# danielSanchezQ/dkg

Hardware: AMD Instinct MI355X
Metric: verified shares/sec (whole node) at n=1024,t=511; full-ceremony wall time (higher is better)
Workload: dtype u32 (GF(2^255-19), Z_l); 1 GPU; one DKG ceremony n=1024, t=511 (share gen + round-2/4 checks + finalise); n=1024, t=511, parallelism=single GPU, verify_streams=2, rounds_2_4_fused=True, degree_split=4, recombination=short lattice multipliers, recombination_addends=affine Niels, stepping_additions=dedicated (complete redo where exceptional)

## Files before the change

dkg_amd/_lib.py:

```python
import ctypes
import os
import sys

HERE = os.path.dirname(os.path.abspath(__file__))
LIB_PATH = os.environ.get("DKG_AMD_LIB", os.path.join(HERE, "libdkg_amd.so"))

DKG_OK = 0
DKG_E_ARG = -1
DKG_E_DECODE = -2
DKG_E_DEVICE = -3
DKG_E_NOMEM = -4
REJECT, ACCEPT, SELF, SKIPPED, MISSING = 0, 1, 2, 3, 4
FIN_OK, FIN_R2_ERROR, FIN_R4_ERROR, FIN_PHASE4_ERROR, FIN_INSUFFICIENT, FIN_PANIC = 0, 1, 2, 3, 4, 5
COMPLAINT_IGNORED, COMPLAINT_NO_PHASE3 = 4, 5

_lib = None


class DkgError(RuntimeError):
    def __init__(self, code, msg=""):
        self.code = code
        names = {DKG_E_ARG: "DKG_E_ARG", DKG_E_DECODE: "DKG_E_DECODE", DKG_E_DEVICE: "DKG_E_DEVICE",
                 DKG_E_NOMEM: "DKG_E_NOMEM"}
        super().__init__(f"{names.get(code, code)}: {msg}")
# ... 130 lines not shown
    L.dkg_ceremony_verify_fetched_proven.argtypes = [p, sz, sz, u8p, u8p, u8p, u8p, u8p, u8p, sz, p, p, u8p, u8p,
                                                     ctypes.POINTER(CeremonyOut), p, p, p]
    L.dkg_ceremony_verify_full_proven.argtypes = [p, sz, sz, u8p, u8p, u8p, u8p, u8p, u8p, sz, p, p, u8p, u8p, sz, p, p,
                                                  u8p, u8p, ctypes.POINTER(CeremonyOut), p, p, p, p, p]
    L.dkg_ceremony_batch_verify_proven.argtypes = [p, sz, sz, sz, u8p, u8p, u8p, u8p, u8p, u8p, sz, p, p, p, u8p, u8p,
                                                   ctypes.POINTER(BatchOut), p, p, p]
    L.dkg_ceremony_batch_verify_full_proven.argtypes = [p, sz, sz, sz, u8p, u8p, u8p, u8p, u8p, u8p, sz, p, p, p, u8p,
                                                        u8p, sz, p, p, p, u8p, u8p, ctypes.POINTER(BatchOut), p, p, p, p,
                                                        p, p, p]
    L.dkg_dealer_coeffs.argtypes = [u8p, ctypes.c_uint32, sz, sz, sz, p, p]
    L.dkg_scalar_sum_device.argtypes = [p, sz, sz, p, p, p]
    L.dkg_point_sum_device.argtypes = [p, sz, p, p, p]
    L.dkg_share_gen_device.argtypes = [p, sz, sz, sz, p, p, p, p, p, p]
    L.dkg_ceremony_shard_recon_device.argtypes = [p, sz, sz, sz, sz, u8p, u8p, u8p, u8p, p, p,
                                                  ctypes.POINTER(ctypes.c_int32)]
    L.dkg_finalise_parties.argtypes = [p, sz, sz, u8p, u8p, u8p, u8p, u8p, u8p, u8p, p, p, p]
    L.dkg_shard_range.argtypes = [sz, sz, sz, ctypes.POINTER(sz), ctypes.POINTER(sz)]
    L.dkg_shard_range.restype = None
    L.dkg_shard_rows.argtypes = [sz, sz]
    L.dkg_shard_rows.restype = sz
    L.dkg_shard_combine_device.argtypes = [p, sz, sz, sz, p, p, p, p, ctypes.POINTER(ShardOutcome)]
    L.dkg_shard_combine_packed_device.argtypes = [p, sz, sz, sz, p, p, p, p, ctypes.POINTER(ShardOutcome)]
    L.dkg_fixed_base_windows.argtypes = []
    L.dkg_key_comb_windows.argtypes = []
    L.dkg_packed_row_words.argtypes = [sz]
    L.dkg_packed_row_words.restype = sz
    L.dkg_decisions_pack_device.argtypes = [p, sz, sz, sz, sz, p, p]
    L.dkg_shard_finalise_device.argtypes = [p, sz, sz, sz, p, p, u8p, ctypes.c_int, p, p, p]
    L.dkg_multi_create.argtypes = [ctypes.POINTER(ctypes.c_int), ctypes.c_int, ctypes.POINTER(p)]
    L.dkg_multi_destroy.argtypes = [p]
    L.dkg_multi_destroy.restype = None
    L.dkg_multi_size.argtypes = [p]
    L.dkg_multi_ctx.argtypes = [p, ctypes.c_int]
    L.dkg_multi_ctx.restype = p
    L.dkg_multi_last_error.argtypes = [p]
    L.dkg_multi_last_error.restype = ctypes.c_char_p
    L.dkg_multi_phase_ms.argtypes = [p, ctypes.c_char_p]
    L.dkg_multi_phase_ms.restype = ctypes.c_double
    L.dkg_multi_env_init.argtypes = [p, sz, sz, u8p, sz, p]
    L.dkg_multi_ceremony_run.argtypes = [p, sz, sz, u8p, u8p, ctypes.POINTER(CeremonyOut)]
    L.dkg_multi_ceremony_run_device.argtypes = [p, sz, sz, ctypes.POINTER(p), ctypes.POINTER(p),
                                                ctypes.POINTER(CeremonyOut)]
    L.dkg_multi_ceremony_verify.argtypes = [p, sz, sz, u8p, u8p, u8p, u8p, ctypes.POINTER(CeremonyOut)]
    _lib = L
    return L


EXPORTED = [
    "dkg_ctx_create", "dkg_ctx_destroy", "dkg_ctx_last_error", "dkg_ctx_phase_ms", "dkg_ctx_set_streams", "dkg_ctx_set_overlap",
    "dkg_device_count", "dkg_env_init",
    "dkg_env_check", "dkg_msm_batch", "dkg_fixed_base_batch", "dkg_poly_eval_batch",
    "dkg_points_valid_batch", "dkg_share_gen", "dkg_verify_pairs", "dkg_verify_receiver",
    "dkg_ctx_set_split", "dkg_ctx_set_stepping", "dkg_ctx_set_field_mode", "dkg_ctx_set_binomial", "dkg_ctx_set_check", "dkg_ctx_last_split", "dkg_ctx_last_split_len", "dkg_ctx_set_verify_mode", "dkg_ctx_fallback_rows", "dkg_split_model_ms", "dkg_split_len",
    "dkg_ctx_set_combine", "dkg_ctx_last_combine", "dkg_ctx_last_binomial", "dkg_ctx_set_addends", "dkg_ctx_set_stepping_formula", "dkg_ctx_stepping_redos", "dkg_ctx_binomial_reruns", "dkg_split_multipliers", "dkg_jsf_digits", "dkg_split_digits",
    "dkg_ctx_clock_probe", "dkg_device_pci_bus_id",
    "dkg_ceremony_run", "dkg_ceremony_verify", "dkg_ceremony_verify_fetched", "dkg_ceremony_run_device", "dkg_ceremony_shard_device",
    "dkg_ceremony_shard_verify_device",
    "dkg_ceremony_batch_device", "dkg_ceremony_batch_verify", "dkg_member_keys", "dkg_enc_randomness",
    "dkg_enc_randomness_device", "dkg_encrypt_shares", "dkg_decrypt_shares", "dkg_ceremony_run_full_device",
    "dkg_ceremony_verify_full", "dkg_misbehaviour_prove", "dkg_complaint1_verify", "dkg_complaint3_verify", "dkg_dealer_coeffs", "dkg_dealer_coeffs_device",
    "dkg_scalar_sum_device", "dkg_point_sum_device", "dkg_ceremony_shard_recon_device", "dkg_finalise_parties",
    "dkg_share_gen_device", "dkg_shard_range", "dkg_shard_rows", "dkg_shard_combine_device",
    "dkg_shard_combine_packed_device", "dkg_packed_row_words", "dkg_fixed_base_windows", "dkg_key_comb_windows", "dkg_decisions_pack_device",
    "dkg_shard_finalise_device", "dkg_multi_create", "dkg_multi_destroy", "dkg_multi_size", "dkg_multi_ctx",
    "dkg_multi_last_error", "dkg_multi_phase_ms", "dkg_multi_env_init", "dkg_multi_ceremony_run",
    "dkg_multi_ceremony_run_device", "dkg_multi_ceremony_verify",
    "dkg_member_keys_batch", "dkg_encrypt_shares_batch", "dkg_decrypt_shares_batch", "dkg_ceremony_batch_full_device",
    "dkg_ceremony_batch_verify_full", "dkg_ctx_set_batch_full_chunk",
    "dkg_complaints_prove", "dkg_complaints_verify", "dkg_ctx_set_complaint_eval", "dkg_ceremony_verify_full_complaints",
    "dkg_complaints3_verify", "dkg_ceremony_verify_fetched_proven", "dkg_ceremony_verify_full_proven",
    "dkg_ceremony_batch_verify_proven", "dkg_ceremony_batch_verify_full_proven",
]
```

dkg_amd/csrc/kernels.h:

```cpp
#pragma once
#include <hip/hip_runtime.h>
#include <stddef.h>
#include <stdint.h>

#include "kernels_decl.inc"
```

dkg_amd/csrc/kernels.hip:

```cpp
#ifdef DKG_FE_ILP
#define dkgk dkgk_ilp
#endif
#include "kernels.h"
#include "split.h"

#include <algorithm>
#include <cmath>
#include "points.h"

namespace dkgk {

constexpr int COMB_WORDS = AFF_WORDS * COMB_ENTRIES;

#ifndef DKG_DECODE_WAVES
#define DKG_DECODE_WAVES 2
#endif
__global__ __launch_bounds__(256, DKG_DECODE_WAVES) void k_decode(const uint32_t* __restrict__ comp, size_t count,
                                                uint32_t* __restrict__ ext, size_t stride,
                                                uint8_t* __restrict__ ok, size_t pm_N, size_t pm_npad,
                                                uint32_t nseg, uint32_t seg, size_t pm_L, size_t pm_pstride) {
  size_t e = (size_t)blockIdx.x * blockDim.x + threadIdx.x;
  if (e >= count) return;
  uint32_t w[8];
  ld_words8(w, comp + 8 * e);
// ... 760 lines not shown
}

void binomial_wave_redo(size_t width, size_t npad, size_t N, const uint32_t* C, uint32_t* e, hipStream_t stream,
                        size_t pieces, size_t pstride, size_t last_len, uint32_t* flags, size_t col_base,
                        size_t dreal, unsigned gw) {
  const int last_off = (last_len && last_len < N) ? (int)(N - last_len) : 0;
  hipLaunchKernelGGL((k_binom_wave<true, false, false>), dim3((unsigned)(width / 64 * pieces)), dim3(64), 0, stream,
                     (int)N, npad, C, e, pstride, (unsigned)(width / 64), (unsigned)(pieces - 1), last_off, nullptr,
                     flags, col_base, dreal, gw ? gw : 64u);
}

uint32_t* binomial(size_t width, size_t npad, size_t N, const uint32_t* C, uint32_t* e0, uint32_t* e1,
                   hipStream_t stream, size_t pieces, size_t pstride, size_t last_len) {
  binom_init(width, npad, N, C, e0, stream, pieces, pstride);
  uint32_t* in = e0;
  uint32_t* out = e1;
  for (size_t r = 1; r < N; r++) {
    binom_step(r, width, npad, N, C, in, out, stream, pieces, pstride, last_len);
    std::swap(in, out);
  }
  return in;
}


__global__ __launch_bounds__(256) void k_to_column_major(size_t width, size_t npad, size_t N,
                                                         const uint32_t* __restrict__ e, uint32_t* __restrict__ eT,
                                                         size_t pstride) {
  __shared__ uint32_t tile[64][65];
  const size_t w = blockIdx.z % PT_WORDS, base = (blockIdx.z / PT_WORDS) * pstride;
  const size_t c0 = (size_t)blockIdx.x * 64, p0 = (size_t)blockIdx.y * 64;
  const size_t S = N * npad;
  const int tx = threadIdx.x & 63, ty = threadIdx.x >> 6;
#pragma unroll
  for (int i = 0; i < 16; i++) {
    const size_t p = p0 + ty + 4 * i, c = c0 + tx;
    if (p < N && c < width) tile[ty + 4 * i][tx] = e[w * S + p * npad + base + c];
  }
  __syncthreads();
#pragma unroll
  for (int i = 0; i < 16; i++) {
    const size_t c = c0 + ty + 4 * i, p = p0 + tx;
    if (p < N && c < width) eT[w * S + (base + c) * N + p] = tile[tx][ty + 4 * i];
  }
}

void to_column_major(size_t width, size_t npad, size_t N, const uint32_t* e, uint32_t* eT, size_t pieces,
                     size_t pstride, hipStream_t stream) {
  if (!width || !N) return;
  hipLaunchKernelGGL(k_to_column_major,
                     dim3((unsigned)((width + 63) / 64), (unsigned)((N + 63) / 64), (unsigned)(pieces * PT_WORDS)),
                     dim3(256), 0, stream, width, npad, N, e, eT, pstride);
}

template <int MAXBS, bool DED, bool PARTS>
__global__ __launch_bounds__(MAXBS) __attribute__((amdgpu_waves_per_eu(4, 4))) void k_stepping(
    size_t ndealers, size_t npad, size_t N, const uint32_t* __restrict__ e, size_t nrecv, size_t pos0, int P,
    const uint32_t* __restrict__ up,
    uint32_t* __restrict__ down,
    uint32_t* __restrict__ R, size_t pstride, size_t Nlive, unsigned piece0, int nseg, int Plast,
    uint32_t* __restrict__ flags, size_t col0, size_t dreal, unsigned gw, uint32_t* __restrict__ Rz, size_t j0,
    size_t j1, const uint32_t* __restrict__ sin, uint32_t* __restrict__ sout, size_t nin, size_t nout) {
  const size_t wg = (size_t)blockIdx.y * gridDim.x + blockIdx.x;
  if (!DED && flags && !flags[wg]) return;
  __shared__ uint32_t cols[PT_WORDS * MAXBS];
  const int l = threadIdx.x, bs = blockDim.x;
  const int Ncol = (nseg - 1) * P + Plast;
  const int slot = l / Ncol, p = l - slot * Ncol;
  const int sg = min(p / P, nseg - 1), q = p - sg * P;
  const int Pseg = sg == nseg - 1 ? Plast : P;
  const size_t dl = (size_t)blockIdx.x * (bs / Ncol) + slot;
  const bool live = slot < bs / Ncol && dl < ndealers;
  const size_t gcol = col0 + dl;
  const bool real = live && (gcol / gw) * 64 + (gcol % gw) % 64 < dreal;
  const size_t d = (blockIdx.y + piece0 + sg) * pstride + dl;
  const size_t S = N * npad;
  const size_t pos = pos0 + q;
  ge_p3 D;
  if (live && pos < Nlive) {
    if (PARTS && j0) pt_load(D, sin, nin * npad, d * nin + pos);
    else pt_load(D, e, S, d * N + pos);
  } else {
    ge_identity(D);
  }
  const bool top_lane = live && (q == Pseg - 1);
  const uint4* upd = (up && live) ? reinterpret_cast<const uint4*>(up + d * nrecv * PT_WORDS) : nullptr;
  uint4* downd = (down && live) ? reinterpret_cast<uint4*>(down + d * nrecv * PT_WORDS) : nullptr;
  uint32_t* mine = cols + l;
  uint32_t* base = cols + (l - q);
  const uint32_t* nbr = base + ((q + 1) % Pseg);
  bool bad = false;
  const size_t jbeg = PARTS ? j0 : 0, jend = PARTS ? j1 : nrecv;
  for (size_t j = jbeg; j < jend; j++) {
    {
      ge_cached c0;
      if (DED) ge_to_cached_ded(c0, D);
      else ge_to_cached(c0, D);
      if (q == 0) {
        if (downd) {
          const uint4* w4 = reinterpret_cast<const uint4*>(&c0);
#pragma unroll
          for (int k = 0; k < PT_WORDS / 4; k++) downd[j * (PT_WORDS / 4) + k] = w4[k];
        }
      } else {
        lds_put_cached(mine, c0, MAXBS);
      }
    }
    if (top_lane && upd) {
      ge_cached u;
      uint4* u4 = reinterpret_cast<uint4*>(&u);
#pragma unroll
      for (int k = 0; k < PT_WORDS / 4; k++) u4[k] = upd[j * (PT_WORDS / 4) + k];
      lds_put_cached(base, u, MAXBS);
    }
    __syncthreads();
    if (live && pos + 1 < Nlive && (q + 1 < Pseg || up) && pos + j < nrecv) {
      if (DED) {
        ge_add_ded_lds(D, D, nbr, MAXBS);
        bad |= real && fe_tight_zero(D.Z);
      } else {
        ge_add_lds(D, D, nbr, false, MAXBS);
      }
    }
    __syncthreads();
    if (live && q == 0 && R) {
      pt_store_aos<DKG_STEP_NT != 0>(R, d * nrecv + j, D);
      if (Rz) {
        uint2* z2 = reinterpret_cast<uint2*>(Rz + (d * nrecv + j) * 10);
#pragma unroll
        for (int k = 0; k < 5; k++) {
          if (DKG_STEP_NT) __builtin_nontemporal_store(D.Z.v[2 * k], reinterpret_cast<uint32_t*>(z2 + k));
          if (DKG_STEP_NT) __builtin_nontemporal_store(D.Z.v[2 * k + 1], reinterpret_cast<uint32_t*>(z2 + k) + 1);
          if (!DKG_STEP_NT) z2[k] = make_uint2(D.Z.v[2 * k], D.Z.v[2 * k + 1]);
        }
      }
    }
  }
  if constexpr (PARTS) {
    if (j1 < nrecv) {
      size_t dd = d;
      int qq = q;
      asm volatile("" : "+v"(dd), "+v"(qq));
      if (live && pos0 + qq < Nlive && pos0 + qq < nout) pt_store(sout, nout * npad, dd * nout + pos0 + qq, D);
    }
  }
  if (DED && bad) flags[wg] = 1u;
}

double step_occupancy(size_t bs, size_t maxbs) {
  const double wgs = std::min(std::floor(160.0 * 1024 / (160.0 * maxbs)), std::floor(16.0 / (bs / 64.0)));
  const double wps = wgs * (bs / 64.0) / 4.0;
  return wps >= 4 ? 1.0 : (wps >= 3 ? 0.85 + 0.15 * (wps - 3) : 0.7);
}

StepShape stepping_shape(size_t N) {
  StepShape sh;
  if (N > 512) {
    sh.nblk = (N + 511) / 512;
    sh.P = (N + sh.nblk - 1) / sh.nblk;
    sh.per = 1;
    sh.bs = (sh.P + 63) / 64 * 64;
    sh.maxbs = 512;
    return sh;
  }
  double best = -1;
  for (size_t maxbs : {256, 192, 512}) {
    if (maxbs < N) continue;
    StepShape o;
    o.nblk = 1;
    o.P = N;
    o.per = maxbs / N;
    o.bs = (o.per * N + 63) / 64 * 64;
    o.maxbs = maxbs;
    const double score = (double)(o.per * N) / o.bs * step_occupancy(o.bs, maxbs);
    if (score > best + 0.02) {
      best = score;
      sh = o;
    }
  }
  return sh;
}

bool stepping_whole_columns(size_t L, size_t pieces, size_t last_len) {
  return pieces > 1 && (pieces - 1) * L + last_len <= 512;
}

double stepping_cycles(size_t cols, size_t N, size_t pieces, size_t last_len, bool whole) {
  const double THR = 4.5, LAT = 8, SIMDS = 1024;
  if (!last_len || last_len > N) last_len = N;
  auto launch = [&](const StepShape& s, double np) {
    const double per_cu = std::min(std::floor(1024.0 / s.maxbs), std::floor(16.0 / (s.bs / 64.0)));
    const double wgs = std::ceil((double)cols / s.per) * np * s.nblk, cap = 256 * per_cu;
    const double rounds = std::ceil(wgs / cap), in_round = wgs / rounds;
    const double w = in_round * (s.bs / 64.0) / SIMDS;
    const double occ = std::min(1.0, std::max(0.7, 0.7 + 0.15 * (w - 2)));
    return rounds * std::max(w * THR / occ, LAT);
  };
  if (whole && stepping_whole_columns(N, pieces, last_len)) return launch(stepping_shape((pieces - 1) * N + last_len), 1);
  const StepShape sh = stepping_shape(N);
  if (sh.nblk > 1 || last_len == N) return launch(sh, (double)pieces);
  return (pieces > 1 ? launch(sh, (double)(pieces - 1)) : 0.0) + launch(stepping_shape(last_len), 1);
}

double stepping_waves_per_simd(size_t cols, size_t N, size_t pieces, size_t last_len, bool whole) {
  if (!last_len || last_len > N) last_len = N;
  const bool wc = whole && stepping_whole_columns(N, pieces, last_len);
  const StepShape s = stepping_shape(wc ? (pieces - 1) * N + last_len : N);
  const double np = wc ? 1.0 : (last_len == N || s.nblk > 1 ? (double)pieces : (double)(pieces - 1));
  const double per_cu = std::min(std::floor(1024.0 / s.maxbs), std::floor(16.0 / (s.bs / 64.0)));
  const double wgs = std::ceil((double)cols / s.per) * np * s.nblk, cap = 256 * per_cu;
  return wgs / std::ceil(wgs / cap) * (s.bs / 64.0) / 1024;
}

constexpr size_t TAIL_MAX_PHASES = 8;
size_t stepping_flag_words(size_t ndealers, size_t pieces) {
  return ndealers * (pieces == 1 ? TAIL_MAX_PHASES : pieces + 1);
}

struct ColReal {
  size_t col0, dreal;
  unsigned gw;
  uint32_t* Rz;
};

template <bool DED, bool PARTS>
void step_launch_p(int maxbs, dim3 grid, dim3 block, hipStream_t stream, size_t ndealers, size_t npad, size_t N,
                   const uint32_t* e, size_t nrecv, size_t pos0, int P, const uint32_t* up, uint32_t* down,
                   uint32_t* R, size_t pstride, size_t Nlive, unsigned piece0, int nseg, int Plast, uint32_t* flags,
                   const ColReal& cr, size_t j0, size_t j1, const uint32_t* sin, uint32_t* sout, size_t nin,
                   size_t nout) {
  if (maxbs == 192)
    hipLaunchKernelGGL((k_stepping<192, DED, PARTS>), grid, block, 0, stream, ndealers, npad, N, e, nrecv, pos0, P,
                       up, down, R, pstride, Nlive, piece0, nseg, Plast, flags, cr.col0, cr.dreal, cr.gw,
                       R ? cr.Rz : nullptr, j0, j1, sin, sout, nin, nout);
  else if (maxbs == 256)
    hipLaunchKernelGGL((k_stepping<256, DED, PARTS>), grid, block, 0, stream, ndealers, npad, N, e, nrecv, pos0, P,
                       up, down, R, pstride, Nlive, piece0, nseg, Plast, flags, cr.col0, cr.dreal, cr.gw,
                       R ? cr.Rz : nullptr, j0, j1, sin, sout, nin, nout);
  else
    hipLaunchKernelGGL((k_stepping<512, DED, PARTS>), grid, block, 0, stream, ndealers, npad, N, e, nrecv, pos0, P,
                       up, down, R, pstride, Nlive, piece0, nseg, Plast, flags, cr.col0, cr.dreal, cr.gw,
                       R ? cr.Rz : nullptr, j0, j1, sin, sout, nin, nout);
}

template <bool DED>
void step_launch(int maxbs, dim3 grid, dim3 block, hipStream_t stream, size_t ndealers, size_t npad, size_t N,
                 const uint32_t* e, size_t nrecv, size_t pos0, int P, const uint32_t* up, uint32_t* down,
                 uint32_t* R, size_t pstride, size_t Nlive, unsigned piece0, int nseg, int Plast, uint32_t* flags,
                 const ColReal& cr, size_t j0, size_t j1, const uint32_t* sin, uint32_t* sout, size_t nin = 0,
                 size_t nout = 0) {
  if (j0 != 0 || j1 != nrecv)
    step_launch_p<DED, true>(maxbs, grid, block, stream, ndealers, npad, N, e, nrecv, pos0, P, up, down, R, pstride,
                             Nlive, piece0, nseg, Plast, flags, cr, j0, j1, sin, sout, nin ? nin : N,
                             nout ? nout : N);
  else
    step_launch_p<DED, false>(maxbs, grid, block, stream, ndealers, npad, N, e, nrecv, pos0, P, up, down, R, pstride,
                              Nlive, piece0, nseg, Plast, flags, cr, 0, nrecv, nullptr, nullptr, N, N);
}

constexpr size_t TAIL_MIN_P = 4;
int stepping_tail_phases(size_t N, size_t nrecv, size_t pieces) {
  if (pieces != 1 || N > 512 || N < 2 * TAIL_MIN_P || 10 * N < 2 * nrecv || nrecv + 1 < N) return 1;
  int k = 1;
  for (size_t P = N / 2; P >= TAIL_MIN_P; P /= 2) k++;
  static_assert(TAIL_MIN_P << (TAIL_MAX_PHASES - 1) >= 512, "flag words of the tail phases");
  return k;
}
size_t stepping_tail_words(size_t ndealers, size_t N) { return PT_WORDS * ndealers * (N / 2); }

bool stepping(size_t ndealers, size_t npad, size_t N, const uint32_t* e, size_t nrecv, uint32_t* R,
              uint32_t* stream_a, uint32_t* stream_b, hipStream_t stream, size_t pieces, size_t pstride,
              size_t last_len, bool whole, uint32_t* flags, size_t col0, size_t dreal, unsigned gw, uint32_t* Rz,
              uint32_t* tail_a, uint32_t* tail_b) {
  if (!ndealers || !nrecv) return true;
  const ColReal cr{col0, dreal, gw ? gw : 64u, Rz};
  if (!last_len || last_len > N) last_len = N;
  size_t foff = 0;
  const size_t fcap = flags ? stepping_flag_words(ndealers, pieces) : 0;
  auto fits = [&](size_t words) { return !flags || foff + words <= fcap; };
  auto run = [&](int maxbs, dim3 grid, dim3 block, size_t pos0, int P, const uint32_t* up, uint32_t* down,
                 uint32_t* Rout, size_t Nlive, unsigned piece0, int nseg, int Plast, uint32_t* f) {
    if (f) {
      step_launch<true>(maxbs, grid, block, stream, ndealers, npad, N, e, nrecv, pos0, P, up, down, Rout, pstride,
                        Nlive, piece0, nseg, Plast, f, cr, 0, nrecv, nullptr, nullptr);
    }
    step_launch<false>(maxbs, grid, block, stream, ndealers, npad, N, e, nrecv, pos0, P, up, down, Rout, pstride,
                       Nlive, piece0, nseg, Plast, f, cr, 0, nrecv, nullptr, nullptr);
  };
  auto launch = [&](const StepShape& s, size_t Nlive, unsigned piece0, size_t np, int nseg, int Plast) {
    const dim3 grid((unsigned)((ndealers + s.per - 1) / s.per), (unsigned)np), block((unsigned)s.bs);
    if (!fits((size_t)grid.x * grid.y)) return false;
    uint32_t* f = flags ? flags + foff : nullptr;
    foff += (size_t)grid.x * grid.y;
    run((int)s.maxbs, grid, block, 0, (int)s.P, nullptr, nullptr, R, Nlive, piece0, nseg, Plast, f);
    return true;
  };
  const int phases = (tail_a && tail_b) ? stepping_tail_phases(N, nrecv, pieces) : 1;
  if (phases > 1) {
    uint32_t* st[2] = {tail_a, tail_b};
    const size_t Nh = N / 2;
    size_t P = N, j0 = 0;
    for (int k = 0; k < phases; k++) {
      const size_t Pn = P / 2, j1 = k + 1 < phases ? nrecv - Pn + 1 : nrecv;
      const StepShape s = stepping_shape(P);
      const dim3 grid((unsigned)((ndealers + s.per - 1) / s.per), 1u), block((unsigned)s.bs);
      if (!fits(grid.x)) return false;
      uint32_t* f = flags ? flags + foff : nullptr;
      foff += grid.x;
      const uint32_t* sin = k ? st[(k - 1) % 2] + col0 * Nh : nullptr;
      uint32_t* sout = k + 1 < phases ? st[k % 2] + col0 * Nh : nullptr;
      for (int pass = f ? 0 : 1; pass < 2; pass++) {
        if (pass == 0)
          step_launch_p<true, true>((int)s.maxbs, grid, block, stream, ndealers, npad, N, e, nrecv, 0, (int)P,
                                    nullptr, nullptr, R, 0, N, 0u, 1, (int)P, f, cr, j0, j1, sin, sout, Nh, Nh);
        else
          step_launch_p<false, true>((int)s.maxbs, grid, block, stream, ndealers, npad, N, e, nrecv, 0, (int)P,
                                     nullptr, nullptr, R, 0, N, 0u, 1, (int)P, f, cr, j0, j1, sin, sout, Nh, Nh);
      }
      P = Pn;
      j0 = j1;
    }
    return true;
  }
  if (whole && stepping_whole_columns(N, pieces, last_len)) {
    StepShape s = stepping_shape((pieces - 1) * N + last_len);
    s.P = N;
    return launch(s, N, 0u, 1, (int)pieces, (int)last_len);
  }
  const StepShape sh = stepping_shape(N);
  if (sh.nblk > 1) {
    auto blocks = [&](size_t Nlive, unsigned piece0, size_t np) {
      const dim3 grid((unsigned)ndealers, (unsigned)np), block((unsigned)sh.bs);
      if (!fits((size_t)grid.x * grid.y)) return false;
      uint32_t* f = flags ? flags + foff : nullptr;
      foff += (size_t)grid.x * grid.y;
      for (int pass = f ? 0 : 1; pass < 2; pass++) {
        uint32_t* up = nullptr;
        for (size_t b = sh.nblk; b-- > 0;) {
          uint32_t* down = b ? ((sh.nblk - 1 - b) % 2 ? stream_b : stream_a) : nullptr;
          if (pass == 0)
            step_launch<true>(512, grid, block, stream, ndealers, npad, N, e, nrecv, b * sh.P, (int)sh.P, up, down,
                              b ? nullptr : R, pstride, Nlive, piece0, 1, (int)sh.P, f, cr, 0, nrecv,
                              nullptr, nullptr);
          else
            step_launch<false>(512, grid, block, stream, ndealers, npad, N, e, nrecv, b * sh.P, (int)sh.P, up, down,
                               b ? nullptr : R, pstride, Nlive, piece0, 1, (int)sh.P, f, cr, 0, nrecv,
// ... 1278 lines not shown
```

dkg_amd/csrc/kernels_decl.inc:

```
namespace dkgk {

void decode_points(const uint32_t* comp, size_t count, uint32_t* ext, size_t stride, uint8_t* ok,
                   hipStream_t stream);
void place_position_major(const uint32_t* src, size_t sstride, size_t D, size_t N, size_t npad, uint32_t* out,
                          hipStream_t stream, int nseg = 1, int seg = 0, size_t L = 0, size_t pstride = 0);
void gather_points(const uint32_t* src, size_t sstride, size_t step, size_t k0, size_t count, uint32_t* dst,
                   size_t dstride, hipStream_t stream);
void decode_position_major(const uint32_t* comp, size_t D, size_t N, size_t npad, uint32_t* out, uint8_t* ok,
                           hipStream_t stream, int nseg = 1, int seg = 0, size_t L = 0, size_t pstride = 0);
void fill_identity(size_t S, uint32_t* out, hipStream_t stream);
void check_both(size_t ndealers, size_t nrecv, size_t dealer0, size_t dealer_base, size_t nmod, const uint32_t* s,
                const uint32_t* sp, const uint32_t* R, const uint32_t* tab_g, const uint32_t* tab_h,
                const uint8_t* dok, uint8_t* dec2, uint8_t* dec4, hipStream_t stream, const uint32_t* scale = nullptr,
                size_t j0 = 0, size_t jn = 0, uint32_t* acc = nullptr);
void encode_points(const uint32_t* ext, size_t stride, size_t count, uint32_t* comp, hipStream_t stream);
void build_comb(const uint32_t* ext, size_t stride, size_t e0, uint32_t* tab, hipStream_t stream, size_t count = 1);
void build_combw(const uint32_t* ext, size_t stride, size_t e0, uint32_t* tab, hipStream_t stream, size_t count = 1);

void commit_position_major(size_t D, size_t N, const uint32_t* a, const uint32_t* b, const uint32_t* tab_g,
                           const uint32_t* tab_h, uint32_t* out, size_t W, size_t L, size_t pstride, uint32_t* A0,
                           size_t A0stride, hipStream_t stream);
void commit(size_t count, const uint32_t* a, const uint32_t* b, const uint32_t* tab_g,
            const uint32_t* tab_h, uint32_t* A_ext, uint32_t* E_ext, hipStream_t stream, size_t stride = 0);
void share_eval(size_t D, size_t n, size_t N, const uint32_t* a, const uint32_t* b, uint32_t* s,
                uint32_t* sp, hipStream_t stream);
void poly_eval(size_t D, size_t N, const uint32_t* coeffs, size_t M, const uint32_t* xs, uint32_t* out,
               hipStream_t stream);

uint32_t* binomial(size_t width, size_t npad, size_t N, const uint32_t* C, uint32_t* e0, uint32_t* e1,
                   hipStream_t stream, size_t pieces = 1, size_t pstride = 0, size_t last_len = 0);
void binom_init(size_t width, size_t npad, size_t N, const uint32_t* C, uint32_t* e0, hipStream_t stream,
                size_t pieces = 1, size_t pstride = 0);
void binom_step(size_t r, size_t width, size_t npad, size_t N, const uint32_t* C, const uint32_t* in, uint32_t* out,
                hipStream_t stream, size_t pieces = 1, size_t pstride = 0, size_t last_len = 0,
                uint32_t* flags = nullptr, size_t col_base = 0, size_t dreal = 0, unsigned gw = 64,
                bool flag_any = false,
                bool nt = false,
                bool il = false);
void binomial_wave_redo(size_t width, size_t npad, size_t N, const uint32_t* C, uint32_t* e, hipStream_t stream,
                        size_t pieces, size_t pstride, size_t last_len, uint32_t* flags, size_t col_base,
                        size_t dreal, unsigned gw);
uint32_t* binomial_wave(size_t width, size_t npad, size_t N, const uint32_t* C, uint32_t* e, hipStream_t stream,
                        size_t pieces = 1, size_t pstride = 0, size_t last_len = 0, uint32_t* eT = nullptr,
                        bool prefetch = false, uint32_t* flags = nullptr, size_t col_base = 0, size_t dreal = 0,
                        unsigned gw = 64);
void binom_step_pair(size_t r, size_t width, size_t npad, size_t N, const uint32_t* C, const uint32_t* in,
                     uint32_t* out, hipStream_t stream, size_t pieces = 1, size_t pstride = 0, size_t last_len = 0);
void to_column_major(size_t width, size_t npad, size_t N, const uint32_t* e, uint32_t* eT, size_t pieces,
                     size_t pstride, hipStream_t stream);
struct StepShape {
  size_t nblk, P, per, bs, maxbs;
};
StepShape stepping_shape(size_t N);
double step_occupancy(size_t bs, size_t maxbs);
bool stepping_whole_columns(size_t L, size_t pieces, size_t last_len);
double stepping_cycles(size_t cols, size_t N, size_t pieces, size_t last_len, bool whole);
double stepping_waves_per_simd(size_t cols, size_t N, size_t pieces, size_t last_len, bool whole);
size_t stepping_flag_words(size_t ndealers, size_t pieces);
bool stepping(size_t ndealers, size_t npad, size_t N, const uint32_t* e, size_t nrecv, uint32_t* R,
              uint32_t* stream_a, uint32_t* stream_b, hipStream_t stream, size_t pieces = 1, size_t pstride = 0,
              size_t last_len = 0, bool whole = true, uint32_t* flags = nullptr, size_t col0 = 0,
              size_t dreal = (size_t)-1, unsigned gw = 64, uint32_t* Rz = nullptr, uint32_t* tail_a = nullptr,
              uint32_t* tail_b = nullptr);
int stepping_tail_phases(size_t N, size_t nrecv, size_t pieces);
size_t stepping_tail_words(size_t ndealers, size_t N);
void combine(size_t width, size_t pstride, size_t pieces, size_t nrecv, const int8_t* digits, const int16_t* top,
             uint32_t* R, hipStream_t stream);
void combine_short(size_t width, size_t pstride, size_t pieces, size_t nrecv, const uint32_t* digits,
                   const int16_t* top, uint32_t* R, hipStream_t stream);
void affine_pieces(size_t width, size_t pstride, size_t pieces, size_t nrecv, const uint32_t* R, uint32_t* A,
                   hipStream_t stream, const uint32_t* Rz = nullptr, size_t j0 = 0, size_t jn = 0);
void combine_short_aff(size_t width, size_t pstride, size_t pieces, size_t nrecv, const uint32_t* digits,
                       const int16_t* top, const uint32_t* A, uint32_t* R, hipStream_t stream, size_t j0 = 0,
                       size_t jn = 0);
void affine_pairs(size_t width, size_t pstride, size_t pieces, size_t nrecv, const uint32_t* R, uint32_t* A,
                  hipStream_t stream, size_t j0 = 0, size_t jn = 0);
constexpr uint32_t JSF_EV_NONE = 0xffu;
constexpr size_t JSF_EV_WORDS = 384;
void combine_short_jsf(size_t width, size_t pstride, size_t pieces, size_t nrecv, const uint32_t* digits,
                       const int16_t* top, const uint32_t* ev, const uint32_t* A, uint32_t* R, hipStream_t stream,
                       size_t j0 = 0, size_t jn = 0);
void check(size_t ndealers, size_t nrecv, size_t dealer_base, size_t recv_base, size_t nmod, int round,
           const uint32_t* s, const uint32_t* sp, const uint32_t* R, const uint32_t* tab_g,
           const uint32_t* tab_h, const uint8_t* dealer_ok, uint8_t* decision, hipStream_t stream,
           const uint32_t* scale = nullptr);
void and_dealer_mask(size_t D, int nseg, int seg, const uint8_t* extra, uint8_t* dok, hipStream_t stream);
void dealer_ok(size_t ndealers, size_t N, const uint8_t* point_ok, uint8_t* ok, hipStream_t stream);
void horner(size_t ndealers, size_t npad, size_t N, const uint32_t* C, uint32_t x0, size_t nrecv, uint32_t* R,
            hipStream_t stream);
void sum_points(size_t count, const uint32_t* pts, size_t stride, const uint8_t* mask, uint32_t* out, size_t ostride,
                size_t col, hipStream_t stream, size_t groups = 1);
void add_points(size_t count, const uint32_t* a, const uint32_t* b, size_t stride, uint32_t* out, hipStream_t stream);
void r4_error(size_t groups, size_t n, size_t t, const uint8_t* dec, const uint8_t* qmask, uint8_t* out,
              hipStream_t stream);
void decision_summary(size_t groups, size_t n, const uint8_t* dec, uint8_t* row_reject, int32_t* complaints,
                      hipStream_t stream);
void apply_skipped(size_t groups, size_t n, uint8_t* dec, const uint8_t* qmask, hipStream_t stream);
void compact_ranks(size_t n, size_t ws, size_t R, size_t width, const void* in, void* out, hipStream_t stream);
void mask_not_and(size_t V, const uint8_t* a, const uint8_t* b, uint8_t* out, hipStream_t stream);
void row_reject(size_t rows, size_t n, const uint8_t* dec, uint8_t* out, hipStream_t stream);
size_t key_comb_words();
int key_comb_windows();
void build_key_combs(const uint32_t* ext, size_t stride, size_t e0, uint32_t* tab, hipStream_t stream,
                     size_t count);
int fixed_base_windows();
void pack_rows(size_t rows, size_t nvalid, size_t n, size_t d0, const uint8_t* dec, uint32_t* out, uint32_t* err,
               hipStream_t stream);
void unpack_ranks(size_t n, size_t ws, size_t R, const uint32_t* in, uint8_t* out, hipStream_t stream);
void from_uniform(const uint32_t* in16, uint32_t* out, hipStream_t stream);
// ... 84 lines not shown
```

dkg_amd/csrc/runtime.hip:

```cpp
#include <hip/hip_runtime.h>

#include <cstdio>
#include <cstdlib>
#include <cstring>
#include <algorithm>
#include <map>
#include <memory>
#include <string>
#include <thread>
#include <unordered_map>
#include <vector>

#include "../../include/dkg_amd.h"
#include "host_crypto.h"
#include "kernels.h"
#include "kernels_ilp.h"

struct dkg_ctx {
  int device = 0;
  hipStream_t stream = nullptr;
  std::string err;
  std::map<std::string, std::pair<void*, size_t>> bufs;
  std::map<std::string, std::pair<void*, size_t>> hbufs;
  uint32_t* tab_g = nullptr;
// ... 283 lines not shown
constexpr size_t SHORT_MAX = 5;
#ifndef DKG_AUTO_SHORT5
#define DKG_AUTO_SHORT5 0
#endif

constexpr int SM_POWERS = 0, SM_NAF = 1, SM_JSF = 2;
bool jsf_built(size_t U) { return U == 2 || U == 4; }

double split_model_ms(size_t cols, size_t n, size_t N, size_t U, size_t L, int short_mult) {
  const double DBL = 1000, ADD = 1400, SIMDS = 1024, THR = 4.5, LAT = 8, LAT_ILP = 6, LAUNCH = 3e-3 * 2.4e6;
  const size_t Lr = last_piece_len(N, U, L), off = L - Lr;
  auto cost = [&](size_t m) {
    uint64_t pos = 0, neg = 0;
    int len = 0;
    for (uint64_t v = m; v; v >>= 1, len++) {
      if (v & 1) {
        if ((v & 3) == 1) {
          pos |= 1ull << len;
          v -= 1;
        } else {
          neg |= 1ull << len;
          v += 1;
        }
      }
    }
    if (len >= 3 && !(((pos | neg) >> (len - 2)) & 1) && ((neg >> (len - 3)) & 1)) {
      pos = (pos & ~(1ull << (len - 1))) | (3ull << (len - 3));
      neg &= ~(1ull << (len - 3));
      len--;
    }
    const int nz = __builtin_popcountll(pos | neg);
    return ADD + (len > 1 ? (len - 1) * DBL + (nz - 1) * ADD : 0.0);
  };

  std::vector<double> pre(L + 1, 0.0);
  for (size_t m = 1; m <= L; m++) pre[m] = pre[m - 1] + cost(m);
  const double waves_col = (double)cols / 64;
  double cyc = 0;
  for (size_t r = 1; r < L; r++) {
    const double work = waves_col * ((U - 1) * pre[r] + (r > off ? pre[r - off] : 0.0)) * THR / SIMDS;
    const double lat = waves_col * U * (r + 1) / SIMDS < 1.5 ? LAT_ILP : LAT;
    cyc += work + cost(r) * lat + LAUNCH;
  }
  if (U > 1) {
    const double bits = 253.0 * (U - 1) / U;
    const bool jsf = short_mult == SM_JSF && jsf_built(U);
    const double adds = jsf ? (U / 2) * bits / 2 + (U % 2) * bits / 3 : U * bits / 3;
    const double per = short_mult && U <= SHORT_MAX ? bits * 950 + adds * ADD + (jsf ? 2 * (U / 2) * 11.75 / 8 * ADD : 0.0)
                                            : (U % 2 == 0 ? 253 * 950 + 85 * ADD : 0.0) +
                                                  ((U + 1) / 2 - 1) * (253 * 950 + 170 * ADD);
    const double waves = (double)cols / 64 * n;
    cyc += std::max(waves * per * THR / SIMDS, per * LAT);
  }
  cyc += n * ADD * dkgk::stepping_cycles(cols, L, U, Lr, stepping_whole_pays(cols, U, L, Lr));
  return cyc / 2.4e6;
}

size_t split_len(size_t cols, size_t n, size_t N, size_t U, int short_mult = SM_JSF) {
  const size_t L1 = (N + U - 1) / U;
  if (U == 1) return L1;
  const size_t L64 = (L1 + 63) / 64 * 64;
  if (L64 == L1 || (U - 1) * L64 >= N) return L1;
  return split_model_ms(cols, n, N, U, L64, short_mult) < split_model_ms(cols, n, N, U, L1, short_mult) ? L64 : L1;
}

double split_model_ms(size_t cols, size_t n, size_t N, size_t U, int short_mult = SM_JSF) {
  return split_model_ms(cols, n, N, U, split_len(cols, n, N, U, short_mult), short_mult);
}

int short_kind(const dkg_ctx* ctx) {
  if (ctx->combine_mode == 1) return SM_POWERS;
  return ctx->combine_mode == 3 || ctx->addend_mode != 0 ? SM_NAF : SM_JSF;
}

size_t choose_split(dkg_ctx* ctx, size_t cols, size_t n, size_t N) {
  if (ctx->split > 0) return std::min<size_t>((size_t)ctx->split, N);
  const int sm = short_kind(ctx);
  const double base = split_model_ms(cols, n, N, 1, sm);
  std::vector<double> ms(17, 0.0);
  double best_ms = base;
  size_t umax = 1;
  for (size_t U = 2; U <= 16; U++) {
    if (N < 64 * U) break;
    ms[U] = split_model_ms(cols, n, N, U, U <= 4 || (ctx->addend_mode == 0 && DKG_AUTO_SHORT5) ? sm : SM_POWERS);
    best_ms = std::min(best_ms, ms[U]);
    umax = U;
  }
  if (!(best_ms < 0.9 * base)) return 1;
  for (size_t U = 2; U <= umax; U++)
    if (ms[U] <= best_ms) return U;
  return 1;
}

void naf_digits(const uint8_t b[32], int8_t* d, int16_t* tp) {
  uint32_t k[9] = {0};
  for (int w = 0; w < 8; w++)
    k[w] = (uint32_t)b[4 * w] | (uint32_t)b[4 * w + 1] << 8 | (uint32_t)b[4 * w + 2] << 16 | (uint32_t)b[4 * w + 3] << 24;
  *tp = -1;
  for (int i = 0; i < 256; i++) {
    d[i] = 0;
    if (!((k[i >> 5] >> (i & 31)) & 1u)) continue;
    int8_t dg = 1;
    if ((k[(i + 1) >> 5] >> ((i + 1) & 31)) & 1u) {
      dg = -1;
      uint64_t carry = 1ull << (i & 31);
      for (int w = i >> 5; carry && w < 9; w++) {
        const uint64_t sum = (uint64_t)k[w] + carry;
// ... 2127 lines not shown
}
int dkg_ctx_binomial_reruns(dkg_ctx* ctx) { return ctx ? ctx->last_binom_rerun : -1; }
int dkg_ctx_set_addends(dkg_ctx* ctx, int mode) {
  if (!ctx || mode < 0 || mode > 1) return DKG_E_ARG;
  ctx->addend_mode = mode;
  return DKG_OK;
}
int dkg_split_multipliers(size_t n, size_t L, int pieces, uint8_t* mag, int8_t* sign) {
  if (!n || !L || pieces < 2 || pieces > (int)SHORT_MAX || !mag || !sign) return DKG_E_ARG;
  try {
    std::vector<uint8_t> m;
    std::vector<int8_t> sg;
    short_vectors(n, L, (size_t)pieces, m, sg, jsf_built((size_t)pieces));
    memcpy(mag, m.data(), m.size());
    memcpy(sign, sg.data(), sg.size());
  } catch (const std::exception&) {
    return DKG_E_NOMEM;
  }
  return DKG_OK;
}
int dkg_jsf_digits(const uint8_t a[32], const uint8_t b[32], int8_t da[256], int8_t db[256], int16_t* top) {
  if (!a || !b || !da || !db || !top) return DKG_E_ARG;
  return dkgh::jsf_digits(a, b, da, db, top) ? DKG_OK : DKG_E_ARG;
}
int dkg_split_digits(size_t n, size_t L, int pieces, int mode, int8_t* digits, int16_t* top) {
  if (!n || !L || pieces < 2 || pieces > (int)SHORT_MAX || mode < 0 || mode > 3 || mode == 1 || !digits || !top)
    return DKG_E_ARG;
  try {
    const size_t K = (size_t)pieces;
    const bool jsf = mode != 3 && jsf_built(K);
    std::vector<uint8_t> m;
    std::vector<int8_t> sg;
    short_vectors(n, L, K, m, sg, jsf);
    std::vector<uint32_t> hd;
    std::vector<int16_t> ht;
    if (!short_digit_words(n, K, jsf, m, sg, hd, ht, nullptr)) return DKG_E_ARG;
    for (size_t j = 0; j < n; j++) {
      top[j] = ht[j];
      for (size_t u = 0; u < K; u++)
        for (size_t b = 0; b < 256; b++)
          digits[(j * K + u) * 256 + b] = (int8_t)(hd[(u / 4) * 256 * n + 256 * j + b] >> (8 * (u % 4)));
    }
  } catch (const std::exception&) {
    return DKG_E_NOMEM;
  }
  return DKG_OK;
}

double dkg_split_model_ms(size_t columns, size_t n, size_t t, int pieces) {
  if (pieces < 1 || t + 1 < (size_t)pieces) return -1;
  return split_model_ms(columns, n, t + 1, (size_t)pieces);
}

size_t dkg_split_len(size_t columns, size_t n, size_t t, int pieces) {
  if (pieces < 1 || t + 1 < (size_t)pieces) return 0;
  return split_len(columns, n, t + 1, (size_t)pieces);
}

int dkg_ctx_set_overlap(dkg_ctx* ctx, int on) {
  if (!ctx) return DKG_E_ARG;
  ctx->overlap = on != 0;
  return DKG_OK;
}

int dkg_env_check(size_t threshold, size_t nr_members) {
  if (nr_members == 0 || !(threshold < (nr_members + 1) / 2)) return DKG_E_ARG;
  return DKG_OK;
}

int dkg_env_init(dkg_ctx* ctx, size_t threshold, size_t nr_members, const uint8_t* ck, size_t ck_len,
                 uint8_t h_out[32]) {
  int rc = dkg_env_check(threshold, nr_members);
  if (rc != DKG_OK) {
    if (ctx) ctx->err = "threshold must be < (nr_members + 1) / 2 (committee.rs:73)";
    return rc;
  }
  return guarded(ctx, [&] {
    uint8_t hash[64];
    dkgh::blake2b(hash, 64, ck, ck_len);
    uint32_t* in = buf<uint32_t>(ctx, "h_in", 64);
    uint32_t* ext = buf<uint32_t>(ctx, "h_ext", PTB);
    uint32_t* comp = buf<uint32_t>(ctx, "h_comp", 32);
    h2d(ctx, in, hash, 64);
    dkgk::from_uniform(in, ext, ctx->stream);
    dkgk::encode_points(ext, 1, 1, comp, ctx->stream);
    check_launch(ctx);
    d2h(ctx, ctx->h, comp, 32);
    sync(ctx);
    bool ok = false;
    comb_for_point(ctx, ctx->h, ctx->tab_h, &ok, ctx->tab_hw);
    if (!ok) return DKG_E_DEVICE;
    ctx->have_h = true;
    ctx->threshold = threshold;
    ctx->nr_members = nr_members;
    if (h_out) memcpy(h_out, ctx->h, 32);
    return DKG_OK;
  });
}

int dkg_msm_batch(dkg_ctx* ctx, size_t B, size_t N, const uint8_t* scalars, const uint8_t* points, uint8_t* out) {
  return guarded(ctx, [&] {
    if (B == 0) return DKG_OK;
    uint32_t* sc = upload_scalars(ctx, "msm_sc", scalars, B * N);
    uint32_t* pc = buf<uint32_t>(ctx, "msm_pc", 32 * B * N);
    uint32_t* pe = buf<uint32_t>(ctx, "msm_pe", PTB * B * N);
    uint8_t* ok = buf<uint8_t>(ctx, "msm_ok", B * N);
// ... 1473 lines not shown
```

include/dkg_amd.h:

```cpp
#ifndef DKG_AMD_H
#define DKG_AMD_H
#include <stddef.h>
#include <stdint.h>

#ifdef __cplusplus
extern "C" {
#endif

#define DKG_OK 0
#define DKG_E_ARG (-1)
#define DKG_E_DECODE (-2)
#define DKG_E_DEVICE (-3)
#define DKG_E_NOMEM (-4)

#define DKG_REJECT 0
#define DKG_ACCEPT 1
#define DKG_SELF 2
#define DKG_SKIPPED 3
#define DKG_MISSING 4

typedef struct dkg_ctx dkg_ctx;

int dkg_ctx_create(int device, dkg_ctx **out);
void dkg_ctx_destroy(dkg_ctx *ctx);
const char *dkg_ctx_last_error(const dkg_ctx *ctx);
double dkg_ctx_phase_ms(const dkg_ctx *ctx, const char *name);
int dkg_ctx_set_streams(dkg_ctx *ctx, int nsub);
int dkg_ctx_set_overlap(dkg_ctx *ctx, int on);
int dkg_ctx_set_split(dkg_ctx *ctx, int pieces);
int dkg_ctx_set_stepping(dkg_ctx *ctx, int mode);
int dkg_ctx_set_field_mode(dkg_ctx *ctx, int mode);
int dkg_ctx_set_binomial(dkg_ctx *ctx, int mode);
int dkg_ctx_set_check(dkg_ctx *ctx, int mode);
int dkg_ctx_set_verify_mode(dkg_ctx *ctx, int mode);
size_t dkg_ctx_fallback_rows(const dkg_ctx *ctx);
int dkg_ctx_last_split(const dkg_ctx *ctx);
size_t dkg_ctx_last_split_len(const dkg_ctx *ctx);
double dkg_split_model_ms(size_t columns, size_t n, size_t t, int pieces);
size_t dkg_split_len(size_t columns, size_t n, size_t t, int pieces);
int dkg_ctx_set_combine(dkg_ctx *ctx, int mode);
int dkg_ctx_last_combine(const dkg_ctx *ctx);
int dkg_ctx_last_binomial(const dkg_ctx *ctx);
int dkg_ctx_set_addends(dkg_ctx *ctx, int mode);
int dkg_ctx_set_stepping_formula(dkg_ctx *ctx, int mode);
long long dkg_ctx_stepping_redos(dkg_ctx *ctx);
int dkg_ctx_binomial_reruns(dkg_ctx *ctx);
int dkg_split_multipliers(size_t n, size_t L, int pieces, uint8_t *mag, int8_t *sign);
int dkg_jsf_digits(const uint8_t a[32], const uint8_t b[32], int8_t da[256], int8_t db[256], int16_t *top);
int dkg_split_digits(size_t n, size_t L, int pieces, int mode, int8_t *digits, int16_t *top);
int dkg_device_count(void);
int dkg_ctx_clock_probe(dkg_ctx *ctx, unsigned iters, double *sclk_mhz, double *busy_ms);
int dkg_device_pci_bus_id(int device, char *buf, int len);

int dkg_env_init(dkg_ctx *ctx, size_t threshold, size_t nr_members, const uint8_t *ck_bytes, size_t ck_len,
                 uint8_t h_out[32]);
int dkg_env_check(size_t threshold, size_t nr_members);

int dkg_msm_batch(dkg_ctx *ctx, size_t B, size_t N, const uint8_t *scalars, const uint8_t *points, uint8_t *out);
int dkg_fixed_base_batch(dkg_ctx *ctx, const uint8_t base[32], size_t count, const uint8_t *scalars, uint8_t *out);
int dkg_poly_eval_batch(dkg_ctx *ctx, size_t D, size_t N, const uint8_t *coeffs, size_t M, const uint32_t *xs,
                        uint8_t *out);
int dkg_points_valid_batch(dkg_ctx *ctx, size_t count, const uint8_t *points, uint8_t *ok);

int dkg_share_gen(dkg_ctx *ctx, size_t D, size_t n, size_t t, const uint8_t *a, const uint8_t *b, uint8_t *E,
                  uint8_t *A, uint8_t *s, uint8_t *s_prime);
int dkg_share_gen_device(dkg_ctx *ctx, size_t D, size_t n, size_t t, const void *d_a, const void *d_b, void *d_E,
                         void *d_A, void *d_s, void *d_s_prime);

int dkg_verify_pairs(dkg_ctx *ctx, size_t n, size_t t, int round, size_t d0, size_t d1, const uint8_t *C,
                     const uint8_t *s, const uint8_t *s_prime, uint8_t *decision);
int dkg_verify_receiver(dkg_ctx *ctx, size_t n, size_t t, int round, size_t j, const uint8_t *C, const uint8_t *s,
                        const uint8_t *s_prime, uint8_t *decision);

typedef struct {
  uint8_t *E, *A;
  uint8_t *s, *s_prime;
  uint8_t *dec2, *dec4;
  uint8_t *qualified;
  uint8_t *r2_error;
  uint8_t *r4_error;
  int32_t *complaints2;
  uint8_t *reconstruct;
  uint8_t *final_share;
  uint8_t *public_share;
  uint8_t mpk[32];
  int32_t n_qualified;
  int32_t phase4_error;
  double ms_round1, ms_round2, ms_round3, ms_round4, ms_finalise, ms_total;
} dkg_ceremony_out;

int dkg_ceremony_run(dkg_ctx *ctx, size_t n, size_t t, const uint8_t *a, const uint8_t *b, dkg_ceremony_out *out);
int dkg_ceremony_verify(dkg_ctx *ctx, size_t n, size_t t, const uint8_t *E, const uint8_t *A, const uint8_t *s,
                        const uint8_t *s_prime, dkg_ceremony_out *out);
int dkg_ceremony_verify_fetched(dkg_ctx *ctx, size_t n, size_t t, const uint8_t *E, const uint8_t *A,
                                const uint8_t *s, const uint8_t *s_prime, const uint8_t *fetched1,
                                const uint8_t *fetched3, dkg_ceremony_out *out);
int dkg_ceremony_run_device(dkg_ctx *ctx, size_t n, size_t t, const void *d_a, const void *d_b,
                            dkg_ceremony_out *out);
// ... 177 lines not shown
```

Measured before the change: 13.34 million verified shares/s.

## Remap stepping-kernel lanes into wave-aligned bands so tail waves retire early

Adds a banded lane mapping for the stepping kernel. Each 64-lane wave holds a contiguous range of positions across all segments, rather than lanes being laid out segment-by-segment. Waves covering high positions run fewer add steps and can retire early, instead of every wave staying live until the last receiver. The split cost model is updated to account for the live-wave fraction. A host lane-map query is exported, and the band path drops the up/down neighbour exchange, so it is only used for equal-length segments without those buffers.

```diff
diff --git a/dkg_amd/_lib.py b/dkg_amd/_lib.py
--- a/dkg_amd/_lib.py
+++ b/dkg_amd/_lib.py
@@ -206,7 +206,7 @@
     "dkg_env_check", "dkg_msm_batch", "dkg_fixed_base_batch", "dkg_poly_eval_batch",
     "dkg_points_valid_batch", "dkg_share_gen", "dkg_verify_pairs", "dkg_verify_receiver",
     "dkg_ctx_set_split", "dkg_ctx_set_stepping", "dkg_ctx_set_field_mode", "dkg_ctx_set_binomial", "dkg_ctx_set_check", "dkg_ctx_last_split", "dkg_ctx_last_split_len", "dkg_ctx_set_verify_mode", "dkg_ctx_fallback_rows", "dkg_split_model_ms", "dkg_split_len",
-    "dkg_ctx_set_combine", "dkg_ctx_last_combine", "dkg_ctx_last_binomial", "dkg_ctx_set_addends", "dkg_ctx_set_stepping_formula", "dkg_ctx_stepping_redos", "dkg_ctx_binomial_reruns", "dkg_split_multipliers", "dkg_jsf_digits", "dkg_split_digits",
+    "dkg_ctx_set_combine", "dkg_ctx_last_combine", "dkg_ctx_last_binomial", "dkg_ctx_set_addends", "dkg_ctx_set_stepping_formula", "dkg_ctx_stepping_redos", "dkg_stepping_lane_map", "dkg_ctx_binomial_reruns", "dkg_split_multipliers", "dkg_jsf_digits", "dkg_split_digits",
     "dkg_ctx_clock_probe", "dkg_device_pci_bus_id",
     "dkg_ceremony_run", "dkg_ceremony_verify", "dkg_ceremony_verify_fetched", "dkg_ceremony_run_device", "dkg_ceremony_shard_device",
     "dkg_ceremony_shard_verify_device",
diff --git a/dkg_amd/csrc/kernels.h b/dkg_amd/csrc/kernels.h
--- a/dkg_amd/csrc/kernels.h
+++ b/dkg_amd/csrc/kernels.h
@@ -3,4 +3,5 @@
 #include <stddef.h>
 #include <stdint.h>
 
+#include "step_map.h"
 #include "kernels_decl.inc"
diff --git a/dkg_amd/csrc/kernels.hip b/dkg_amd/csrc/kernels.hip
--- a/dkg_amd/csrc/kernels.hip
+++ b/dkg_amd/csrc/kernels.hip
@@ -836,7 +836,7 @@
                      dim3(256), 0, stream, width, npad, N, e, eT, pstride);
 }
 
-template <int MAXBS, bool DED, bool PARTS>
+template <int MAXBS, bool DED, bool PARTS, bool BAND = false>
 __global__ __launch_bounds__(MAXBS) __attribute__((amdgpu_waves_per_eu(4, 4))) void k_stepping(
     size_t ndealers, size_t npad, size_t N, const uint32_t* __restrict__ e, size_t nrecv, size_t pos0, int P,
     const uint32_t* __restrict__ up,
@@ -849,8 +849,14 @@
   __shared__ uint32_t cols[PT_WORDS * MAXBS];
   const int l = threadIdx.x, bs = blockDim.x;
   const int Ncol = (nseg - 1) * P + Plast;
-  const int slot = l / Ncol, p = l - slot * Ncol;
-  const int sg = min(p / P, nseg - 1), q = p - sg * P;
+  int slot, sg, q, nxt = 0;
+  if constexpr (BAND) {
+    const StepLane m = step_band_lane(l, 64 / (bs / P), bs);
+    slot = m.seg / nseg, sg = m.seg - slot * nseg, q = m.q, nxt = m.next;
+  } else {
+    const int p = l % Ncol;
+    slot = l / Ncol, sg = min(p / P, nseg - 1), q = p - sg * P;
+  }
   const int Pseg = sg == nseg - 1 ? Plast : P;
   const size_t dl = (size_t)blockIdx.x * (bs / Ncol) + slot;
   const bool live = slot < bs / Ncol && dl < ndealers;
@@ -871,7 +877,7 @@
   uint4* downd = (down && live) ? reinterpret_cast<uint4*>(down + d * nrecv * PT_WORDS) : nullptr;
   uint32_t* mine = cols + l;
   uint32_t* base = cols + (l - q);
-  const uint32_t* nbr = base + ((q + 1) % Pseg);
+  const uint32_t* nbr = BAND ? cols + nxt : base + ((q + 1) % Pseg);
   bool bad = false;
   const size_t jbeg = PARTS ? j0 : 0, jend = PARTS ? j1 : nrecv;
   for (size_t j = jbeg; j < jend; j++) {
@@ -880,7 +886,7 @@
       if (DED) ge_to_cached_ded(c0, D);
       else ge_to_cached(c0, D);
       if (q == 0) {
-        if (downd) {
+        if (!BAND && downd) {
           const uint4* w4 = reinterpret_cast<const uint4*>(&c0);
 #pragma unroll
           for (int k = 0; k < PT_WORDS / 4; k++) downd[j * (PT_WORDS / 4) + k] = w4[k];
@@ -889,7 +895,7 @@
         lds_put_cached(mine, c0, MAXBS);
       }
     }
-    if (top_lane && upd) {
+    if (!BAND && top_lane && upd) {
       ge_cached u;
       uint4* u4 = reinterpret_cast<uint4*>(&u);
 #pragma unroll
@@ -897,7 +903,7 @@
       lds_put_cached(base, u, MAXBS);
     }
     __syncthreads();
-    if (live && pos + 1 < Nlive && (q + 1 < Pseg || up) && pos + j < nrecv) {
+    if (live && pos + 1 < Nlive && (q + 1 < Pseg || (!BAND && up)) && pos + j < nrecv) {
       if (DED) {
         ge_add_ded_lds(D, D, nbr, MAXBS);
         bad |= real && fe_tight_zero(D.Z);
@@ -968,21 +974,36 @@
   return pieces > 1 && (pieces - 1) * L + last_len <= 512;
 }
 
-double stepping_cycles(size_t cols, size_t N, size_t pieces, size_t last_len, bool whole) {
+double step_live_share(const StepShape& s, size_t P, size_t nseg, size_t Plast, size_t nrecv) {
+  if (!nrecv || s.nblk > 1) return 1.0;
+  const int B = step_band((int)s.bs, (int)P, (int)nseg, (int)Plast);
+  const size_t Ncol = (nseg - 1) * P + Plast, waves = s.bs / 64;
+  double steps = 0;
+  for (size_t w = 0; w < waves; w++) {
+    size_t p0 = B ? w * B : P;
+    for (size_t l = 64 * w; !B && l < 64 * w + 64; l++) p0 = std::min(p0, (l % Ncol) % P);
+    steps += nrecv > p0 ? (double)(nrecv - p0) : 0.0;
+  }
+  return steps / ((double)waves * nrecv);
+}
+
+double stepping_cycles(size_t cols, size_t N, size_t pieces, size_t last_len, bool whole, size_t nrecv) {
   const double THR = 4.5, LAT = 8, SIMDS = 1024;
   if (!last_len || last_len > N) last_len = N;
-  auto launch = [&](const StepShape& s, double np) {
+  auto launch = [&](const StepShape& s, double np, size_t P, size_t nseg, size_t Plast) {
     const double per_cu = std::min(std::floor(1024.0 / s.maxbs), std::floor(16.0 / (s.bs / 64.0)));
     const double wgs = std::ceil((double)cols / s.per) * np * s.nblk, cap = 256 * per_cu;
     const double rounds = std::ceil(wgs / cap), in_round = wgs / rounds;
     const double w = in_round * (s.bs / 64.0) / SIMDS;
     const double occ = std::min(1.0, std::max(0.7, 0.7 + 0.15 * (w - 2)));
-    return rounds * std::max(w * THR / occ, LAT);
+    return rounds * std::max(w * THR / occ * step_live_share(s, P, nseg, Plast, nrecv), LAT);
   };
-  if (whole && stepping_whole_columns(N, pieces, last_len)) return launch(stepping_shape((pieces - 1) * N + last_len), 1);
+  if (whole && stepping_whole_columns(N, pieces, last_len))
+    return launch(stepping_shape((pieces - 1) * N + last_len), 1, N, pieces, last_len);
   const StepShape sh = stepping_shape(N);
-  if (sh.nblk > 1 || last_len == N) return launch(sh, (double)pieces);
-  return (pieces > 1 ? launch(sh, (double)(pieces - 1)) : 0.0) + launch(stepping_shape(last_len), 1);
+  if (sh.nblk > 1 || last_len == N) return launch(sh, (double)pieces, sh.P, 1, sh.P);
+  return (pieces > 1 ? launch(sh, (double)(pieces - 1), sh.P, 1, sh.P) : 0.0) +
+         launch(stepping_shape(last_len), 1, last_len, 1, last_len);
 }
 
 double stepping_waves_per_simd(size_t cols, size_t N, size_t pieces, size_t last_len, bool whole) {
@@ -1041,6 +1062,25 @@
                               Nlive, piece0, nseg, Plast, flags, cr, 0, nrecv, nullptr, nullptr, N, N);
 }
 
+template <bool DED>
+void step_launch_band(int maxbs, dim3 grid, dim3 block, hipStream_t stream, size_t ndealers, size_t npad, size_t N,
+                      const uint32_t* e, size_t nrecv, int P, uint32_t* R, size_t pstride, size_t Nlive,
+                      unsigned piece0, int nseg, uint32_t* flags, const ColReal& cr) {
+  uint32_t* Rz = R ? cr.Rz : nullptr;
+  if (maxbs == 192)
+    hipLaunchKernelGGL((k_stepping<192, DED, false, true>), grid, block, 0, stream, ndealers, npad, N, e, nrecv, 0, P,
+                       nullptr, nullptr, R, pstride, Nlive, piece0, nseg, P, flags, cr.col0, cr.dreal, cr.gw, Rz, 0,
+                       nrecv, nullptr, nullptr, N, N);
+  else if (maxbs == 256)
+    hipLaunchKernelGGL((k_stepping<256, DED, false, true>), grid, block, 0, stream, ndealers, npad, N, e, nrecv, 0, P,
+                       nullptr, nullptr, R, pstride, Nlive, piece0, nseg, P, flags, cr.col0, cr.dreal, cr.gw, Rz, 0,
+                       nrecv, nullptr, nullptr, N, N);
+  else
+    hipLaunchKernelGGL((k_stepping<512, DED, false, true>), grid, block, 0, stream, ndealers, npad, N, e, nrecv, 0, P,
+                       nullptr, nullptr, R, pstride, Nlive, piece0, nseg, P, flags, cr.col0, cr.dreal, cr.gw, Rz, 0,
+                       nrecv, nullptr, nullptr, N, N);
+}
+
 constexpr size_t TAIL_MIN_P = 4;
 int stepping_tail_phases(size_t N, size_t nrecv, size_t pieces) {
   if (pieces != 1 || N > 512 || N < 2 * TAIL_MIN_P || 10 * N < 2 * nrecv || nrecv + 1 < N) return 1;
@@ -1075,6 +1115,14 @@
     if (!fits((size_t)grid.x * grid.y)) return false;
     uint32_t* f = flags ? flags + foff : nullptr;
     foff += (size_t)grid.x * grid.y;
+    if (step_band((int)s.bs, (int)s.P, nseg, Plast)) {
+      if (f)
+        step_launch_band<true>((int)s.maxbs, grid, block, stream, ndealers, npad, N, e, nrecv, (int)s.P, R, pstride,
+                               Nlive, piece0, nseg, f, cr);
+      step_launch_band<false>((int)s.maxbs, grid, block, stream, ndealers, npad, N, e, nrecv, (int)s.P, R, pstride,
+                              Nlive, piece0, nseg, f, cr);
+      return true;
+    }
     run((int)s.maxbs, grid, block, 0, (int)s.P, nullptr, nullptr, R, Nlive, piece0, nseg, Plast, f);
     return true;
   };
diff --git a/dkg_amd/csrc/kernels_decl.inc b/dkg_amd/csrc/kernels_decl.inc
--- a/dkg_amd/csrc/kernels_decl.inc
+++ b/dkg_amd/csrc/kernels_decl.inc
@@ -54,7 +54,7 @@
 StepShape stepping_shape(size_t N);
 double step_occupancy(size_t bs, size_t maxbs);
 bool stepping_whole_columns(size_t L, size_t pieces, size_t last_len);
-double stepping_cycles(size_t cols, size_t N, size_t pieces, size_t last_len, bool whole);
+double stepping_cycles(size_t cols, size_t N, size_t pieces, size_t last_len, bool whole, size_t nrecv = 0);
 double stepping_waves_per_simd(size_t cols, size_t N, size_t pieces, size_t last_len, bool whole);
 size_t stepping_flag_words(size_t ndealers, size_t pieces);
 bool stepping(size_t ndealers, size_t npad, size_t N, const uint32_t* e, size_t nrecv, uint32_t* R,
diff --git a/dkg_amd/csrc/runtime.hip b/dkg_amd/csrc/runtime.hip
--- a/dkg_amd/csrc/runtime.hip
+++ b/dkg_amd/csrc/runtime.hip
@@ -359,7 +359,7 @@
     const double waves = (double)cols / 64 * n;
     cyc += std::max(waves * per * THR / SIMDS, per * LAT);
   }
-  cyc += n * ADD * dkgk::stepping_cycles(cols, L, U, Lr, stepping_whole_pays(cols, U, L, Lr));
+  cyc += n * ADD * dkgk::stepping_cycles(cols, L, U, Lr, stepping_whole_pays(cols, U, L, Lr), n);
   return cyc / 2.4e6;
 }
 
@@ -2593,6 +2593,15 @@
   return split_model_ms(columns, n, t + 1, (size_t)pieces);
 }
 
+int dkg_stepping_lane_map(int lanes, int seg_len, int nseg, int last_len, int lane, int out[3]) {
+  if (lanes <= 0 || lanes % 64 || lanes > 512 || lane < 0 || lane >= lanes || !out) return -1;
+  const int B = step_band(lanes, seg_len, nseg, last_len);
+  if (!B) return 0;
+  const StepLane m = step_band_lane(lane, B, lanes);
+  out[0] = m.seg, out[1] = m.q, out[2] = m.next;
+  return B;
+}
+
 size_t dkg_split_len(size_t columns, size_t n, size_t t, int pieces) {
   if (pieces < 1 || t + 1 < (size_t)pieces) return 0;
   return split_len(columns, n, t + 1, (size_t)pieces);
diff --git a/dkg_amd/csrc/step_map.h b/dkg_amd/csrc/step_map.h
--- /dev/null
+++ b/dkg_amd/csrc/step_map.h
@@ -0,0 +1,30 @@
+#pragma once
+
+#if defined(__HIPCC__) || defined(__CUDACC__)
+#define DKG_STEP_MAP_FN __host__ __device__ inline
+#else
+#define DKG_STEP_MAP_FN inline
+#endif
+
+struct StepLane {
+  int seg;
+  int q;
+  int next;
+};
+
+DKG_STEP_MAP_FN int step_band(int bs, int P, int nseg, int Plast) {
+  if (P <= 0 || nseg <= 0 || Plast != P || bs % P) return 0;
+  const int S = bs / P;
+  if (S < 2 || S > 64 || 64 % S || S % nseg) return 0;
+  return 64 / S;
+}
+
+DKG_STEP_MAP_FN StepLane step_band_lane(int l, int B, int bs) {
+  const int w = l >> 6, s = (l & 63) / B, r = l % B;
+  StepLane m;
+  m.seg = s;
+  m.q = w * B + r;
+  m.next = r + 1 < B ? l + 1 : l + 65 - B;
+  if (m.next >= bs) m.next = s * B;
+  return m;
+}
diff --git a/include/dkg_amd.h b/include/dkg_amd.h
--- a/include/dkg_amd.h
+++ b/include/dkg_amd.h
@@ -44,6 +44,7 @@
 int dkg_ctx_set_addends(dkg_ctx *ctx, int mode);
 int dkg_ctx_set_stepping_formula(dkg_ctx *ctx, int mode);
 long long dkg_ctx_stepping_redos(dkg_ctx *ctx);
+int dkg_stepping_lane_map(int lanes, int seg_len, int nseg, int last_len, int lane, int out[3]);
 int dkg_ctx_binomial_reruns(dkg_ctx *ctx);
 int dkg_split_multipliers(size_t n, size_t L, int pieces, uint8_t *mag, int8_t *sign);
 int dkg_jsf_digits(const uint8_t a[32], const uint8_t b[32], int8_t da[256], int8_t db[256], int16_t *top);
```

New measurement: 13.49 million verified shares/s (median of 6 runs). 1.2% higher.
